# ctxnn/GenConViT

Measured on AMD Instinct MI355X. Metric: frames/sec (224x224, ed+vae forward), higher is better.
Workload: dtype f16

## Files before the change

genconvit_amd/_lib.py:

```python
from __future__ import annotations

import ctypes
import ctypes.util
import json
import os
import threading

_HERE = os.path.dirname(os.path.abspath(__file__))
LIB_PATH = os.environ.get("GCV_LIB_PATH") or os.path.join(_HERE, "lib", "libgenconvit_hip.so")

GCV_F32, GCV_BF16, GCV_F16 = 0, 1, 2
ACT_NONE, ACT_RELU, ACT_GELU, ACT_LEAKY = 0, 1, 2, 3
A_PLAIN, A_IM2COL3_POOL, A_IM2COL3_S2 = 0, 1, 2
EPI_BIAS_ACT, EPI_RESID, EPI_POOL4, EPI_CONVT, EPI_SPLITK = 0, 1, 2, 3, 4

c_void_p, c_int, c_int64, c_float, c_char_p, c_size_t = (ctypes.c_void_p, ctypes.c_int, ctypes.c_int64,
                                                         ctypes.c_float, ctypes.c_char_p, ctypes.c_size_t)


class TensorDesc(ctypes.Structure):
    _fields_ = [("name", c_char_p), ("data", c_void_p), ("numel", c_int64), ("on_device", c_int)]


class GemmArgs(ctypes.Structure):
# ... 95 lines not shown
    "gcv_k_gelu_bwd": (c_int, [c_int, c_void_p, c_void_p, c_void_p, c_void_p, c_int, c_int, c_void_p]),
    "gcv_k_dw_ln_bwd": (c_int, [c_int, c_void_p, c_void_p, c_void_p, c_void_p, c_void_p, c_void_p, c_void_p, c_int, c_int,
                                c_int, c_float, c_void_p]),
    "gcv_k_dw_dgrad_res": (c_int, [c_void_p, c_void_p, c_void_p, c_int, c_int, c_int, c_void_p]),
    "gcv_k_down_ln_bwd": (c_int, [c_int, c_void_p, c_void_p, c_void_p, c_void_p, c_void_p, c_int, c_int, c_int, c_float,
                                  c_void_p]),
    "gcv_k_cam2": (c_int, [c_int, c_int, c_int, c_void_p, c_void_p, c_void_p, c_void_p, c_int, c_int, c_int, c_int, c_int,
                           c_int, c_void_p, c_void_p, c_void_p, c_int, c_void_p]),
    "gcv_k_fused_mlp": (c_int, [c_int, c_int, c_void_p, c_void_p, c_void_p, c_void_p, c_void_p, c_void_p, c_void_p,
                                c_void_p, c_int, c_void_p]),
    "gcv_k_fused_mlp_lnp": (c_int, [c_int, c_int, c_void_p, c_void_p, c_void_p, c_void_p, c_void_p, c_void_p, c_void_p,
                                    c_void_p, c_void_p, c_float, c_int, c_void_p, c_void_p, c_void_p, c_void_p, c_void_p,
                                    c_int, c_void_p]),
    "gcv_k_fused_mlp_timed": (c_int, [c_int, c_int, c_void_p, c_void_p, c_void_p, c_void_p, c_void_p, c_void_p,
                                      c_void_p, c_void_p, c_int, c_int, c_void_p, c_void_p]),
}

_lib = None
_lock = threading.Lock()


class GenConViTHipError(RuntimeError):
    pass


def _preload_hip_runtime():
    cands = []
    try:
        import torch
        cands.append(os.path.join(os.path.dirname(torch.__file__), "lib", "libamdhip64.so"))
# ... 779 lines not shown
```

genconvit_amd/csrc/api.hip:

```cpp
#include "../../include/genconvit_hip.h"

#include <dlfcn.h>

#include <cstdio>
#include <cstdlib>
#include <cstring>
#include <map>
#include <mutex>
#include <set>
#include <sstream>
#include <vector>

#include "cam.h"
#include "cam_bwd.h"
#include "cnx_mlp.h"
#include "gemm.h"
#include "kernels.h"
#include "net.h"

namespace gcv {
static thread_local std::string g_err;
void set_error(const std::string& msg) { g_err = msg; }
const char* get_error() { return g_err.c_str(); }

// ... 132 lines not shown
    GCV_REQUIRE(w[i].name && w[i].data && w[i].numel > 0, "tensor descriptor with null name/data");
    m[w[i].name] = TensorRef{(const float*)w[i].data, w[i].numel, w[i].on_device != 0};
  }
  return 0;
}

template <typename T> struct MlpTestRunner {
  hipStream_t s;
  const char* only;
  template <class F> int run(const char* tag, double, double, F&& f) { return only && std::strcmp(tag, only) ? 0 : f(); }
  int gemm(const char*, const GemmArgs& g, int a_mode, int epi) { return launch_gemm<T>(g, a_mode, epi, s); }
};
template <typename T>
static int k_mlp_dispatch(int C, const void* x, const void* w1, const float* b1, const float* w2_f32, const float* b2,
                          const float* gamma, const void* resid, void* out, int M, hipStream_t s, int iters = 0,
                          float* ms = nullptr, const LnpSpec* lnp = nullptr) {
  struct Bufs {
    hipStream_t s;
    std::vector<void*> p;
    ~Bufs() { (void)hipStreamSynchronize(s); for (void* q : p) (void)hipFree(q); }
  } bufs{s, {}};
  auto alloc = [&](size_t n) -> void* {
    void* q = nullptr;
    if (hipMalloc(&q, n) != hipSuccess) return nullptr;
    bufs.p.push_back(q);
    return q;
  };
  struct Ev {
    hipEvent_t e = nullptr;
    ~Ev() { if (e) (void)hipEventDestroy(e); }
  };
  CnxMlpW<T> w;
  w.kind = mlp_kind(sizeof(T), C);
  GCV_REQUIRE(w.kind != MlpKind::Gemm, "the fused MLP kernels cover C = 96, 192 and 384");
  w.w1 = (const T*)w1; w.b1 = b1; w.b2 = b2; w.gamma = gamma;
  GCV_TRY(pack_cnx_mlp<T>(w, C, w2_f32, alloc, s));
  T* hidden = w.kind == MlpKind::Pair384 ? (T*)alloc(mlp_pair_hidden_bytes(M, C)) : nullptr;
  GCV_REQUIRE(hidden || w.kind != MlpKind::Pair384, "hipMalloc of the hidden tensor");
  auto launch = [&](const char* only) {
    MlpTestRunner<T> r{s, only};
    return launch_cnx_mlp<T>(r, w, C, (const T*)x, (const T*)resid, (T*)out, hidden, M, lnp, s);
  };
  auto timed = [&](const char* only, float* avg) -> int {
    if (iters <= 0) return launch(only);
    Ev e0, e1;
    GCV_CHECK_HIP(hipEventCreate(&e0.e));
    GCV_CHECK_HIP(hipEventCreate(&e1.e));
    GCV_TRY(launch(only));
    GCV_CHECK_HIP(hipEventRecord(e0.e, s));
    for (int i = 0; i < iters; ++i) GCV_TRY(launch(only));
    GCV_CHECK_HIP(hipEventRecord(e1.e, s));
    GCV_CHECK_HIP(hipEventSynchronize(e1.e));
    float t = 0.0f;
    GCV_CHECK_HIP(hipEventElapsedTime(&t, e0.e, e1.e));
    if (avg) *avg = t / (float)iters;
    return 0;
// ... 619 lines not shown
  return launch_face_quality((const unsigned char*)frames_u8_nhwc, nframes, H, W, boxes5, n, grid, out8, (hipStream_t)s);
}

int gcv_face_signature(const void* frames_u8_nhwc, int nframes, int H, int W, const int* boxes5, int n, void* sig384,
                       gcv_stream s) {
  GCV_REQUIRE(n <= 0 || (frames_u8_nhwc && boxes5 && sig384), "face signature: null pointer");
  return launch_face_signature((const unsigned char*)frames_u8_nhwc, nframes, H, W, boxes5, n, (unsigned char*)sig384,
                               (hipStream_t)s);
}

int gcv_sig_link(const void* sig384, const int* owner, int n, int tracks, uint32_t* out_u32, gcv_stream s) {
  GCV_REQUIRE(n <= 0 || tracks <= 0 || (sig384 && owner && out_u32), "sig link: null pointer");
  return launch_sig_link((const unsigned char*)sig384, owner, n, tracks, out_u32, (hipStream_t)s);
}

int gcv_k_fused_mlp(int dtype, int C, const void* x, const void* w1, const float* b1, const float* w2_f32,
                    const float* b2, const float* gamma, const void* resid, void* out, int M, gcv_stream s) {
  GCV_REQUIRE(dtype == GCV_F16 || dtype == GCV_BF16, "the MLP kernels are built for 16-bit storage");
  if (dtype == GCV_F16) return k_mlp_dispatch<half_t>(C, x, w1, b1, w2_f32, b2, gamma, resid, out, M, (hipStream_t)s);
  return k_mlp_dispatch<bf16_t>(C, x, w1, b1, w2_f32, b2, gamma, resid, out, M, (hipStream_t)s);
}

int gcv_k_fused_mlp_lnp(int dtype, int C, const void* x, const void* w1, const float* b1, const float* w2_f32,
                        const float* b2, const float* gamma, const void* resid, const float* ln_w, const float* ln_b,
                        float eps, int nseg, const int* tok0, const int* hw, const int* wd, const int* out0, void* out, int M,
                        gcv_stream s) {
  GCV_REQUIRE(dtype == GCV_F16 || dtype == GCV_BF16, "the MLP kernels are built for 16-bit storage");
  LnpSpec l;
  GCV_TRY(lnp_from_tables(l, C, M, ln_w, ln_b, eps, nseg, tok0, hw, wd, out0));
  if (dtype == GCV_F16)
    return k_mlp_dispatch<half_t>(C, x, w1, b1, w2_f32, b2, gamma, resid, out, M, (hipStream_t)s, 0, nullptr, &l);
  return k_mlp_dispatch<bf16_t>(C, x, w1, b1, w2_f32, b2, gamma, resid, out, M, (hipStream_t)s, 0, nullptr, &l);
}

int gcv_k_fused_mlp_timed(int dtype, int C, const void* x, const void* w1, const float* b1, const float* w2_f32,
                          const float* b2, const float* gamma, const void* resid, void* out, int M, int iters,
                          float* ms3, gcv_stream s) {
  GCV_REQUIRE(dtype == GCV_F16 || dtype == GCV_BF16, "the MLP kernels are built for 16-bit storage");
  GCV_REQUIRE(iters >= 1 && ms3 != nullptr, "gcv_k_fused_mlp_timed: iters >= 1 and a float[3] for the averages");
  if (dtype == GCV_F16)
    return k_mlp_dispatch<half_t>(C, x, w1, b1, w2_f32, b2, gamma, resid, out, M, (hipStream_t)s, iters, ms3);
  return k_mlp_dispatch<bf16_t>(C, x, w1, b1, w2_f32, b2, gamma, resid, out, M, (hipStream_t)s, iters, ms3);
}

}
```

genconvit_amd/csrc/cnx_mlp.h:

```cpp
#pragma once
#include "fused_mlp.h"
#include "gemm.h"
#include "mlp_pair.h"
#include "xs_mlp.h"

namespace gcv {

enum class MlpKind {
  Gemm,
  Fused96,
  Xs192,
  Pair384,
};
static inline MlpKind mlp_kind(size_t tsize, int C) {
  if (tsize != 2) return MlpKind::Gemm;
  if (C == 96) return MlpKind::Fused96;
  if (C == 192) return MlpKind::Xs192;
  if (C == 384) return MlpKind::Pair384;
  return MlpKind::Gemm;
}

template <typename T> struct CnxMlpW {
  MlpKind kind = MlpKind::Gemm;
  const T* w1 = nullptr;
// ... 51 lines not shown
    t += (int64_t)n[s] * h[s] * wd[s];
    o += (int64_t)n[s] * (h[s] / 2) * (wd[s] / 2);
    even = even && h[s] % 2 == 0 && wd[s] % 2 == 0;
  }
  return even && lnp_supported(kind, C, M);
}
template <typename A> static void set_lnp(A& a, const LnpSpec& l) {
  a.lnp_w = l.w; a.lnp_b = l.b; a.lnp_eps = l.eps; a.lnp_nseg = l.nseg;
  for (int s = 0; s < l.nseg; ++s) {
    a.lnp_tok0[s] = l.tok0[s]; a.lnp_hw[s] = l.hw[s]; a.lnp_wd[s] = l.wd[s]; a.lnp_out0[s] = l.out0[s];
  }
}

template <typename T, class R>
int launch_cnx_mlp(R& r, const CnxMlpW<T>& w, int C, const T* x, const T* resid, T* out, T* hidden, int M,
                   const LnpSpec* lnp, hipStream_t s) {
  GCV_REQUIRE(!lnp || lnp_supported(w.kind, C, M), "LN-patchify epilogue of an MLP kind without one");
  if constexpr (sizeof(T) == 2) {
    const double fused_flops = 16.0 * M * C * (double)C, fused_bytes = 3.0 * sizeof(T) * (double)M * C + 16.0 * C * C;
    switch (w.kind) {
      case MlpKind::Gemm: break;
      case MlpKind::Fused96: {
        MlpArgs a{x, w.w1, w.b1, w.w2c, w.b2, w.gamma, resid, out, M};
        if (lnp) set_lnp(a, *lnp);
        return r.run("cnx.fused_mlp", fused_flops, fused_bytes, [&] { return launch_fused_mlp<T>(a, C, s); });
      }
      case MlpKind::Xs192: {
        XsMlpArgs a{x, w.wp, w.b1, w.b2, w.gamma, resid, out, M};
        if (lnp) set_lnp(a, *lnp);
        return r.run("cnx.fused_mlp", fused_flops, fused_bytes, [&] { return launch_xs_mlp<T>(a, C, s); });
      }
      case MlpKind::Pair384: {
        MlpPairArgs a{x, w.w1f, w.b1, w.w2f, w.b2, w.gamma, resid, out, hidden, M};
        GCV_TRY(r.run("cnx.pw1_gelu", 8.0 * M * C * (double)C, sizeof(T) * (5.0 * M * C + 4.0 * C * C),
                      [&] { return launch_xs_pw1<T>(a, C, s); }));
        return r.run("cnx.pw2_scale_res", 8.0 * M * C * (double)C, sizeof(T) * (6.0 * M * C + 4.0 * C * C),
                     [&] { return launch_pw2f<T>(a, C, s); });
      }
    }
  }
  GemmArgs g1{};
  g1.A = x; g1.lda = C; g1.Wt = w.w1; g1.C = hidden; g1.ldc = 4 * C; g1.bias = w.b1;
  g1.M = M; g1.N = 4 * C; g1.K = C; g1.act = ACT_GELU; g1.splitk = 1;
  GCV_TRY(r.gemm("cnx.pw1_gelu", g1, A_PLAIN, EPI_BIAS_ACT));
  GemmArgs g2{};
// ... 7 lines not shown
```

genconvit_amd/csrc/diag/diag.h:

```cpp
#pragma once

#ifndef GCV_XS_ABLATE
#define GCV_XS_ABLATE 0
#endif
#ifndef GCV_P2_ABLATE
#define GCV_P2_ABLATE 0
#endif
#ifndef GCV_XM_ABLATE
#define GCV_XM_ABLATE 0
#endif
#ifndef GCV_MLP_ABLATE
#define GCV_MLP_ABLATE 0
#endif
#ifndef GCV_GLDS_ABLATE
#define GCV_GLDS_ABLATE 0
#endif
#ifndef GCV_DWR_ABLATE
#define GCV_DWR_ABLATE 0
#endif
#ifndef GCV_DWM_ABLATE
#define GCV_DWM_ABLATE 0
#endif
#ifndef GCV_XS_STAMPS
#define GCV_XS_STAMPS 0
#endif
#ifndef GCV_XS_STAMP_WAVE
#define GCV_XS_STAMP_WAVE 0
#endif
#ifndef GCV_P2_STAMPS
#define GCV_P2_STAMPS 0
#endif
#ifndef GCV_P2_STAMP_WAVE
#define GCV_P2_STAMP_WAVE 0
#endif
#ifndef GCV_XM_STAMPS
#define GCV_XM_STAMPS 0
// ... 97 lines not shown
```

genconvit_amd/csrc/fused_mlp.h:

```cpp
#pragma once
#include "gemm.h"

namespace gcv {


struct MlpArgs {
  const void* X;
  const void* W1;
  const float* b1;
  const void* W2c;
  const float* b2;
  const float* gamma;
  const void* resid;
  void* out;
  int M;
  const float* lnp_w = nullptr;
  const float* lnp_b = nullptr;
  float lnp_eps = 0.0f;
  int lnp_nseg = 0;
  int lnp_tok0[4] = {0, 0, 0, 0};
  int lnp_hw[4] = {1, 1, 1, 1};
  int lnp_wd[4] = {1, 1, 1, 1};
  int lnp_out0[4] = {0, 0, 0, 0};
};
// ... 214 lines not shown
    for (int i = 0; i < 12; ++i) {
      const int idx = lane + 64 * i;
      const int row = idx / 24, pc = idx - row * 24;
      const int64_t mm = m_wave + row;
      const f32x4 v = *(const f32x4*)(sC + row * 100 + 4 * pc);
      t4 o4;
#pragma unroll
      for (int e = 0; e < 4; ++e) o4[e] = from_f<T>(v[e] + to_f(rres[i][e]));
      if (mm < a.M) *(t4*)(Op + mm * C + half * 96 + 4 * pc) = o4;
    }
    __syncthreads();
  }
  GCV_STAMP(6);
}

template <typename T> int launch_fused_mlp(const MlpArgs& a, int C, hipStream_t s);
template <typename T> int launch_pack_w2_chunks(const float* w2_dev, T* out, int C, hipStream_t s);

}
```

genconvit_amd/csrc/fused_mlp_bf16.hip:

```cpp
#include "fused_mlp_impl.h"
namespace gcv {
template int launch_fused_mlp<bf16_t>(const MlpArgs&, int, hipStream_t);
template int launch_pack_w2_chunks<bf16_t>(const float*, bf16_t*, int, hipStream_t);
}
```

genconvit_amd/csrc/fused_mlp_f16.hip:

```cpp
#include "fused_mlp_impl.h"
namespace gcv {
template int launch_fused_mlp<half_t>(const MlpArgs&, int, hipStream_t);
template int launch_pack_w2_chunks<half_t>(const float*, half_t*, int, hipStream_t);
}

GCV_MLP_STAMP_READER
```

genconvit_amd/csrc/fused_mlp_impl.h:

```cpp
#pragma once
#include "fused_mlp.h"
#include "fused_mlp_res.h"

namespace gcv {

template <typename T>
__global__ void __launch_bounds__(256) pack_w2_chunks_kernel(const float* __restrict__ w2, T* __restrict__ out, int C,
                                                             int HC) {
  const int64_t total = (int64_t)C * 4 * C;
  const int64_t i = (int64_t)blockIdx.x * 256 + threadIdx.x;
  if (i >= total) return;
  const int p = (int)(i % HC);
  const int64_t t = i / HC;
  const int o = (int)(t % C);
  const int ch = (int)(t / C);
  const int kk = p >> 4, h = (p >> 3) & 1, jj = p & 7;
  const int hid = 16 * kk + 8 * (jj >> 2) + 4 * h + (jj & 3);
  out[i] = from_f<T>(w2[(int64_t)o * 4 * C + ch * HC + hid]);
}

template <typename T> int launch_pack_w2_chunks(const float* w2_dev, T* out, int C, hipStream_t s) {
  constexpr int HC = kMlpHC;
  GCV_REQUIRE((4 * C) % HC == 0, "hidden width must be a multiple of the chunk");
  const int64_t total = (int64_t)C * 4 * C;
  hipLaunchKernelGGL((pack_w2_chunks_kernel<T>), dim3((unsigned)cdiv64(total, 256)), dim3(256), 0, s, w2_dev, out, C, HC);
  GCV_CHECK_HIP(hipGetLastError());
  return 0;
}

template <typename T, int C, int NW> static int launch_mlp_c(const MlpArgs& a, hipStream_t s) {
  constexpr int SMEM = MlpSmem<T, C, NW>::bytes;
  GCV_ENSURE_LDS((fused_mlp_kernel<T, C, NW>), SMEM);
  hipLaunchKernelGGL((fused_mlp_kernel<T, C, NW>), dim3(cdiv(a.M, NW * 32)), dim3(NW * 64), SMEM, s, a);
  GCV_CHECK_HIP(hipGetLastError());
  return 0;
}

template <typename T> int launch_fused_mlp_res(const MlpArgs& a, hipStream_t s) {
  constexpr int SMEM = MlpResSmem::bytes;
  GCV_ENSURE_LDS((fused_mlp_res_kernel<T>), SMEM);
  constexpr int nw = 8;
  const int wave_tiles = cdiv(a.M, 32);
  const int nwg = cdiv(wave_tiles, nw) < 256 ? cdiv(wave_tiles, nw) : 256;
  if (a.lnp_nseg > 0) {
    GCV_REQUIRE(a.lnp_w && a.lnp_b && a.lnp_nseg <= 4, "fused MLP: LN-patchify epilogue arguments");
    GCV_ENSURE_LDS((fused_mlp_res_kernel<T, true>), SMEM);
    hipLaunchKernelGGL((fused_mlp_res_kernel<T, true>), dim3(nwg), dim3(64 * nw), SMEM, s, a);
  } else {
    hipLaunchKernelGGL((fused_mlp_res_kernel<T>), dim3(nwg), dim3(64 * nw), SMEM, s, a);
  }
  GCV_CHECK_HIP(hipGetLastError());
  return 0;
}

template <typename T> int launch_fused_mlp(const MlpArgs& a, int C, hipStream_t s) {
  GCV_REQUIRE(a.M > 0 && a.X && a.W1 && a.W2c && a.b1 && a.b2 && a.gamma && a.resid && a.out, "fused MLP: null argument");
  if (fused_mlp_res_applies(C, a.M)) return launch_fused_mlp_res<T>(a, s);
  GCV_REQUIRE(a.lnp_nseg == 0, "fused MLP: the LN-patchify epilogue exists in the LDS-resident kernel only");
  GCV_REQUIRE(C == 96, "fused MLP kernels of this file: C = 96");
  return launch_mlp_c<T, 96, 4>(a, s);
}

}
```

genconvit_amd/csrc/fused_mlp_res.h:

```cpp
#pragma once
#include "fused_mlp.h"

namespace gcv {

struct MlpResSmem {
  static constexpr int kRow = 192;
  static constexpr int kW1 = 0;
  static constexpr int kW2 = 384 * kRow;
  static constexpr int kB1 = 2 * 384 * kRow;
  static constexpr int kB2 = kB1 + 384 * 4;
  static constexpr int kG = kB2 + 96 * 4;
  static constexpr int kCtr = kG + 96 * 4;
  static constexpr int kLn = kCtr + 16;
  static constexpr int bytes = kLn + 2 * 96 * 4;
};

__device__ __forceinline__ int mlp_res_swz(int row, int k16) { return (k16 & ~3) | ((k16 & 3) ^ ((row >> 2) & 3)); }

template <typename T, bool LNP = false>
__global__ void __launch_bounds__(512, 1) fused_mlp_res_kernel(const MlpArgs a) {
  static_assert(sizeof(T) == 2, "fused MLP is built for 16-bit storage");
  constexpr int C = 96, HC = 96, NG = 12;
  constexpr int KP1 = C / 16;
  constexpr int NO = C / 32;
// ... 25 lines not shown
      sf[i] = i < 384 ? a.b1[i] : (i < 480 ? a.b2[i - 384] : a.gamma[i - 480]);
    if (tid == 0) *reinterpret_cast<int*>(smem + MlpResSmem::kCtr) = (int)blockDim.x >> 6;
    if (LNP) {
      float* sl = reinterpret_cast<float*>(smem + MlpResSmem::kLn);
      for (int i = tid; i < 192; i += (int)blockDim.x) sl[i] = i < 96 ? a.lnp_w[i] : a.lnp_b[i - 96];
    }
  }
  __syncthreads();
  RES_STAMP(11);

  const T* __restrict__ Xp = (const T*)a.X;
  const T* Rp = (const T*)a.resid;
  T* Op = (T*)a.out;
  typedef T t4 __attribute__((ext_vector_type(4)));

  const int ntiles = (a.M + 31) / 32;
  const int nwaves = (int)blockDim.x >> 6;
  const int stride = (int)gridDim.x * nwaves;
  const int key = (lr >> 2) & 3;
  const int rowoff = lr * ROW;

  u32x4 xf[KP1];
  auto load_x = [&](int tile) {
    const int64_t mm = (int64_t)tile * 32 + lr;
    const int64_t mmc = (GCV_MLP_ABLATE & 8) ? (int64_t)lr : (mm < a.M ? mm : (int64_t)a.M - 1);
#pragma unroll
    for (int p = 0; p < KP1; ++p) xf[p] = *(const u32x4*)(Xp + mmc * C + 16 * p + 8 * lh);
  };
  int* const ctr = reinterpret_cast<int*>(smem + MlpResSmem::kCtr);
  auto slot_tile = [&](int q) { return (int)blockIdx.x * nwaves + (q % nwaves) + (q / nwaves) * stride; };
  auto next_slot = [&]() {
    int q = 0;
    if (lane == 0) q = atomicAdd(ctr, 1);
    return __builtin_amdgcn_readfirstlane(q);
  };
  if (slot_tile(wave) < ntiles) load_x(slot_tile(wave));
  int titer = 0;
  for (int tile = slot_tile(wave), tile_next = 0; tile < ntiles; tile = tile_next, ++titer) {
    tile_next = slot_tile(next_slot());
    if (titer == 2) GCV_STAMP(0);
#if GCV_MLP_STAMPS
    if (titer == 2 && blockIdx.x < 64 && threadIdx.x == 0) gcv_mlp_stamps[blockIdx.x * 16 + 8] = __builtin_amdgcn_s_memrealtime();
#endif
    const int64_t m = (int64_t)tile * 32 + lr;
    const int64_t mc = m < a.M ? m : (int64_t)a.M - 1;
// ... 209 lines not shown
        }
        auto sx = __builtin_amdgcn_permlane32_swap(pk[0].x, pk[1].x, false, false);
        auto sy = __builtin_amdgcn_permlane32_swap(pk[0].y, pk[1].y, false, false);
        const u32x4 w = {sx[0], sy[0], sx[1], sy[1]};
        const int n16 = 32 * o + 8 * q + 8 * lh;
        if (m < a.M && (!(GCV_MLP_ABLATE & 8) || w[0] == 0x12345u)) *(u32x4*)(Op + m * C + n16) = w;
      }
    if (titer == 2) GCV_STAMP(6);
#if GCV_MLP_STAMPS
    if (titer == 2 && blockIdx.x < 64 && threadIdx.x == 0) gcv_mlp_stamps[blockIdx.x * 16 + 9] = __builtin_amdgcn_s_memrealtime();
#endif
  }
  RES_STAMP(12);
}

template <typename T> int launch_fused_mlp_res(const MlpArgs& a, hipStream_t s);

}
```

genconvit_amd/csrc/xs_mlp.h:

```cpp
#pragma once
#include <type_traits>

#include "gemm.h"

namespace gcv {

struct XsMlpArgs {
  const void* X;
  const void* Wp;
  const float* b1;
  const float* b2;
  const float* gamma;
  const void* resid;
  void* out;
  int M;
  const float* lnp_w = nullptr;
  const float* lnp_b = nullptr;
  float lnp_eps = 0.0f;
  int lnp_nseg = 0;
  int lnp_tok0[4] = {0, 0, 0, 0};
  int lnp_hw[4] = {1, 1, 1, 1};
  int lnp_wd[4] = {1, 1, 1, 1};
  int lnp_out0[4] = {0, 0, 0, 0};
};
// ... 25 lines not shown
  static constexpr int NKC = 4 * C / 32;
  static constexpr int D = C == 96 ? 10 : 6;
  static constexpr int PPW = 3;
  static constexpr int NLW = NM / PPW;
  static constexpr int kB1 = D * REC;
  static constexpr int kBG = kB1 + 4 * C * 4;
  static constexpr int kLn = kBG + 2 * C * 4;
  static constexpr int bytes = kLn + 2 * C * 4;
  static constexpr int NSB = NM / 4;
};


#define GCV_XM_WAIT(N) asm volatile("s_waitcnt vmcnt(%0)\n\ts_barrier" ::"n"(N) : "memory")

template <typename T, int C, bool LNP = false>
__global__ void __launch_bounds__(512, 2) xs_mlp_kernel(const XsMlpArgs a, const int npass) {
  static_assert(sizeof(T) == 2, "16-bit storage");
  static_assert(C == 96 || C == 192, "narrow ConvNeXt stages");
  typedef XsMlpCfg<C> CF;
  constexpr int KP1 = CF::KP1, NO = CF::NO, NM = CF::NM, REC = CF::REC, NKC = CF::NKC, D = CF::D, PPW = CF::PPW;
  constexpr int NLW = CF::NLW, NSB = CF::NSB;
  static_assert(D >= 6 && NKC % 2 == 0, "ring: four live chunks and two incoming; passes are whole pairs of steps");
  typedef T t4 __attribute__((ext_vector_type(4)));

  extern __shared__ __attribute__((aligned(16))) unsigned char smem[];

  const int tid = threadIdx.x;
  const int lane = tid & 63;
  const int wave = __builtin_amdgcn_readfirstlane(tid >> 6);
  const int lr = lane & 31, lh = lane >> 5;

  const int my_passes = (npass - (int)blockIdx.x + (int)gridDim.x - 1) / (int)gridDim.x;
  if (my_passes <= 0) return;

  {
    float* sf = reinterpret_cast<float*>(smem + CF::kB1);
    for (int i = tid; i < 6 * C; i += 512) sf[i] = i < 4 * C ? a.b1[i] : (i < 5 * C ? a.b2[i - 4 * C] : a.gamma[i - 5 * C]);
    if (LNP) {
      float* sl = reinterpret_cast<float*>(smem + CF::kLn);
      for (int i = tid; i < 2 * C; i += 512) sl[i] = i < C ? a.lnp_w[i] : a.lnp_b[i - C];
    }
  }
  __syncthreads();

  const bool loader = wave < NLW;
  const unsigned char* const wsrc = (const unsigned char*)a.Wp + wave * 1024;
  const unsigned lane16 = (unsigned)lane * 16u;
  int gw = 0, slot_w = 0;
  auto issue = [&]() {
    if (loader) {
      const unsigned char* src = wsrc + (int64_t)gw * REC;
      unsigned char* dst = smem + slot_w * REC + wave * 1024;
#pragma unroll
      for (int i = 0; i < PPW; ++i)
        __builtin_amdgcn_global_load_lds((const __attribute__((address_space(1))) void*)(src + i * NLW * 1024 + lane16),
                                         (__attribute__((address_space(3))) void*)(dst + i * NLW * 1024), 16, 0, 0);
    }
    gw = gw + 1 == NKC ? 0 : gw + 1;
    slot_w = slot_w + 1 == D ? 0 : slot_w + 1;
  };
// ... 5 lines not shown
  const float* const sG_ = sB2_ + C;
  const T* __restrict__ Xp = (const T*)a.X;
  const T* Rp = (const T*)a.resid;
  T* Op = (T*)a.out;

  int slot1 = 0;
  auto slot_dec = [&](int s, int k) { return s - k < 0 ? s - k + D : s - k; };

  u32x4 xf[KP1];
  auto load_x = [&](int64_t mc) {
    const T* xp = Xp + mc * C + 8 * lh;
#pragma unroll
    for (int p = 0; p < KP1; ++p)
      asm volatile("global_load_dwordx4 %0, %1, off offset:%2" : "=v"(xf[p]) : "v"(xp), "n"(p * 32) : "memory");
  };
  auto row_of = [&](int it) { return ((int64_t)((int)blockIdx.x + it * (int)gridDim.x) * 8 + wave) * 32 + lr; };
  {
    const int64_t m0 = row_of(0);
    load_x(m0 < a.M ? m0 : (int64_t)a.M - 1);
  }
  XM_STAMP(0);

  for (int it = 0; it < my_passes; ++it) {
    const int64_t m = row_of(it);
    const int64_t mc = m < a.M ? m : (int64_t)a.M - 1;
    asm volatile("s_waitcnt vmcnt(0)" ::: "memory");
#pragma unroll
    for (int p = 0; p < KP1; ++p) asm volatile("" : "+v"(xf[p]));

    f32x16 acc2[NO];
#pragma unroll
    for (int o = 0; o < NO; ++o)
#pragma unroll
      for (int r = 0; r < 16; ++r) acc2[o][r] = 0.0f;

    GeluH16::State<4> gst;
    float gx[8];
    auto gelu_a = [&](const f32x16& acc, int half) {
#pragma unroll
      for (int c = 0; c < 8; ++c) gx[c] = acc[8 * half + c];
// ... 198 lines not shown
            const int q = 2 * pr + d;
            const int n = 32 * o + 8 * q;
            const f32x4 bv = *(const f32x4*)(sB2 + n);
            const f32x4 gv = *(const f32x4*)(sG + n);
            t4 o4;
#pragma unroll
            for (int e = 0; e < 4; ++e) o4[e] = from_f<T>(fmaf(acc2[o][4 * q + e] + bv[e], gv[e], to_f(rq[d][e])));
            pk[d] = __builtin_bit_cast(uint2, o4);
          }
          const auto sx = __builtin_amdgcn_permlane32_swap(pk[0].x, pk[1].x, false, false);
          const auto sy = __builtin_amdgcn_permlane32_swap(pk[0].y, pk[1].y, false, false);
          const u32x4 w = {sx[0], sy[0], sx[1], sy[1]};
          if (m < a.M) *(u32x4*)(Op + m * C + 32 * o + 16 * pr + 8 * lh) = w;
        }
    }
    if (it + 1 < my_passes) {
      const int64_t mn = row_of(it + 1);
      load_x(mn < a.M ? mn : (int64_t)a.M - 1);
    }
    if (it == 0) XM_STAMP(5);
  }
  asm volatile("s_waitcnt vmcnt(0)" ::: "memory");
  XM_STAMP(6);
}

template <typename T> int launch_xs_mlp(const XsMlpArgs& a, int C, hipStream_t s);
template <typename T, typename S> int launch_pack_xs_mlp(const T* w1, const S* w2, T* out, int C, hipStream_t s);
static inline bool xs_mlp_supported(int C) { return C == 192; }
static inline size_t xs_mlp_packed_elems(int C) { return (size_t)(4 * C / 32) * (size_t)(C / 16 + 2 * (C / 32)) * 512; }

}
```

genconvit_amd/csrc/xs_mlp_bf16.hip:

```cpp
#include "xs_mlp_impl.h"
namespace gcv {
template int launch_xs_mlp<bf16_t>(const XsMlpArgs&, int, hipStream_t);
template int launch_pack_xs_mlp<bf16_t, bf16_t>(const bf16_t*, const bf16_t*, bf16_t*, int, hipStream_t);
template int launch_pack_xs_mlp<bf16_t, float>(const bf16_t*, const float*, bf16_t*, int, hipStream_t);
}
```

genconvit_amd/csrc/xs_mlp_f16.hip:

```cpp
#include "xs_mlp_impl.h"
namespace gcv {
template int launch_xs_mlp<half_t>(const XsMlpArgs&, int, hipStream_t);
template int launch_pack_xs_mlp<half_t, half_t>(const half_t*, const half_t*, half_t*, int, hipStream_t);
template int launch_pack_xs_mlp<half_t, float>(const half_t*, const float*, half_t*, int, hipStream_t);
}

GCV_XM_STAMP_READER
```

genconvit_amd/csrc/xs_mlp_impl.h:

```cpp
#pragma once
#include "xs_mlp.h"

namespace gcv {

template <typename T, typename S> int launch_pack_xs_mlp(const T* w1, const S* w2, T* out, int C, hipStream_t s) {
  GCV_REQUIRE(xs_mlp_supported(C), "pack_xs_mlp: unsupported C");
  const int64_t total = (int64_t)xs_mlp_packed_elems(C);
  hipLaunchKernelGGL((pack_xs_mlp_kernel<T, S>), dim3((unsigned)cdiv64(total, 256)), dim3(256), 0, s, w1, w2, out, C);
  GCV_CHECK_HIP(hipGetLastError());
  return 0;
}

template <typename T, int C> static int launch_xs_mlp_c(const XsMlpArgs& a, hipStream_t s) {
  constexpr int SMEM = XsMlpCfg<C>::bytes;
  GCV_ENSURE_LDS((xs_mlp_kernel<T, C>), SMEM);
  const int npass = cdiv(a.M, 256);
  const int nwg = npass < 256 ? npass : 256;
  if (a.lnp_nseg > 0) {
    GCV_REQUIRE(a.lnp_w && a.lnp_b && a.lnp_nseg <= 4, "xs MLP: LN-patchify epilogue arguments");
    GCV_ENSURE_LDS((xs_mlp_kernel<T, C, true>), SMEM);
    hipLaunchKernelGGL((xs_mlp_kernel<T, C, true>), dim3(nwg), dim3(512), SMEM, s, a, npass);
    GCV_CHECK_HIP(hipGetLastError());
    return 0;
  }
  hipLaunchKernelGGL((xs_mlp_kernel<T, C>), dim3(nwg), dim3(512), SMEM, s, a, npass);
  GCV_CHECK_HIP(hipGetLastError());
  return 0;
}

template <typename T> int launch_xs_mlp(const XsMlpArgs& a, int C, hipStream_t s) {
  GCV_REQUIRE(a.M > 0 && a.X && a.Wp && a.b1 && a.b2 && a.gamma && a.resid && a.out, "xs MLP: null argument");
  auto al = [](const void* p) { return (reinterpret_cast<uintptr_t>(p) & 15u) == 0; };
  GCV_REQUIRE(al(a.X) && al(a.Wp) && al(a.resid) && al(a.out), "xs MLP: operands must be 16-byte aligned");
  if (C == 192) return launch_xs_mlp_c<T, 192>(a, s);
  set_error("xs MLP is built for C = 192");
  return -3;
}

}
```

include/genconvit_hip.h:

```cpp
#ifndef GENCONVIT_HIP_H
#define GENCONVIT_HIP_H

#include <stddef.h>
#include <stdint.h>

#ifdef __cplusplus
extern "C" {
#endif

#if defined(GCV_BUILD)
#pragma GCC visibility push(default)
#endif

typedef struct gcv_handle gcv_handle;
typedef void* gcv_stream;

enum { GCV_F32 = 0, GCV_BF16 = 1, GCV_F16 = 2 };
enum { GCV_CONVNEXT_TINY = 0, GCV_CONVNEXT_LARGE = 1 };
enum { GCV_LARGE_MAX_BATCH = 256 };
enum { GCV_ACT_NONE = 0, GCV_ACT_RELU = 1, GCV_ACT_GELU = 2, GCV_ACT_LEAKY = 3 };

typedef struct {
  const char* name;
  const void* data;
// ... 162 lines not shown
int gcv_k_down_ln_bwd(int dtype, const void* x, const float* ln_w, const float* dP, const float* inv, float* dA2,
                      int nimg, int side2, int C2, float eps, gcv_stream s);
int gcv_k_cam2(int dtype, int C2, int npass, const void* A0, const void* A1, const float* dA0, const float* dA1,
               int side0, int side1, int off0, int off1, int cam_ld, int up_pass, float* cam, float* cam224, float* alpha,
               int B, gcv_stream s);

int gcv_k_fused_mlp(int dtype, int C, const void* x, const void* w1, const float* b1, const float* w2_f32,
                    const float* b2, const float* gamma, const void* resid, void* out, int M, gcv_stream s);
int gcv_k_fused_mlp_lnp(int dtype, int C, const void* x, const void* w1, const float* b1, const float* w2_f32,
                        const float* b2, const float* gamma, const void* resid, const float* ln_w, const float* ln_b,
                        float eps, int nseg, const int* tok0, const int* hw, const int* wd, const int* out0, void* out, int M,
                        gcv_stream s);
int gcv_k_fused_mlp_timed(int dtype, int C, const void* x, const void* w1, const float* b1, const float* w2_f32,
                          const float* b2, const float* gamma, const void* resid, void* out, int M, int iters,
                          float* ms3, gcv_stream s);

#if defined(GCV_BUILD)
#pragma GCC visibility pop
#endif

#ifdef __cplusplus
}
#endif
#endif
```

Baseline: 18580.

## Spread MLP tail tiles across workgroups with a shared tile-walk scheme

Adds a shared tile-walk helper that both fused MLP kernels (C=96 LDS-resident and C=192 xs) use to map tiles to workgroup waves. The partial last round is spread across more workgroups instead of being packed onto the first few, so the tail imbalance shrinks. In the xs kernel, waves that finish early keep issuing weight-stream loads so the shared loader pipeline stays in step. It also exposes max-workgroup entry points and a walk-inspection API for testing. The cost is extra per-kernel index arithmetic and idle loader loops.

```diff
diff --git a/genconvit_amd/_lib.py b/genconvit_amd/_lib.py
--- a/genconvit_amd/_lib.py
+++ b/genconvit_amd/_lib.py
@@ -133,6 +133,12 @@
                                     c_int, c_void_p]),
     "gcv_k_fused_mlp_timed": (c_int, [c_int, c_int, c_void_p, c_void_p, c_void_p, c_void_p, c_void_p, c_void_p,
                                       c_void_p, c_void_p, c_int, c_int, c_void_p, c_void_p]),
+    "gcv_k_fused_mlp_wg": (c_int, [c_int, c_int, c_void_p, c_void_p, c_void_p, c_void_p, c_void_p, c_void_p, c_void_p,
+                                   c_void_p, c_int, c_int, c_void_p]),
+    "gcv_k_fused_mlp_lnp_wg": (c_int, [c_int, c_int, c_void_p, c_void_p, c_void_p, c_void_p, c_void_p, c_void_p, c_void_p,
+                                       c_void_p, c_void_p, c_float, c_int, c_void_p, c_void_p, c_void_p, c_void_p, c_void_p,
+                                       c_int, c_int, c_void_p]),
+    "gcv_mlp_walk": (c_int, [c_int, c_int, c_int, c_void_p, c_void_p, c_int]),
 }
 
 _lib = None
diff --git a/genconvit_amd/csrc/api.hip b/genconvit_amd/csrc/api.hip
--- a/genconvit_amd/csrc/api.hip
+++ b/genconvit_amd/csrc/api.hip
@@ -170,7 +170,7 @@
 template <typename T>
 static int k_mlp_dispatch(int C, const void* x, const void* w1, const float* b1, const float* w2_f32, const float* b2,
                           const float* gamma, const void* resid, void* out, int M, hipStream_t s, int iters = 0,
-                          float* ms = nullptr, const LnpSpec* lnp = nullptr) {
+                          float* ms = nullptr, const LnpSpec* lnp = nullptr, int max_wg = kMlpMaxWg) {
   struct Bufs {
     hipStream_t s;
     std::vector<void*> p;
@@ -195,7 +195,7 @@
   GCV_REQUIRE(hidden || w.kind != MlpKind::Pair384, "hipMalloc of the hidden tensor");
   auto launch = [&](const char* only) {
     MlpTestRunner<T> r{s, only};
-    return launch_cnx_mlp<T>(r, w, C, (const T*)x, (const T*)resid, (T*)out, hidden, M, lnp, s);
+    return launch_cnx_mlp<T>(r, w, C, (const T*)x, (const T*)resid, (T*)out, hidden, M, lnp, s, max_wg);
   };
   auto timed = [&](const char* only, float* avg) -> int {
     if (iters <= 0) return launch(only);
@@ -845,23 +845,56 @@
   return launch_sig_link((const unsigned char*)sig384, owner, n, tracks, out_u32, (hipStream_t)s);
 }
 
+int gcv_k_fused_mlp_wg(int dtype, int C, const void* x, const void* w1, const float* b1, const float* w2_f32,
+                       const float* b2, const float* gamma, const void* resid, void* out, int M, int max_wg, gcv_stream s) {
+  GCV_REQUIRE(dtype == GCV_F16 || dtype == GCV_BF16, "the MLP kernels are built for 16-bit storage");
+  GCV_REQUIRE(max_wg >= 1 && max_wg <= kMlpMaxWg, "fused MLP: max_wg outside 1 .. 256");
+  if (dtype == GCV_F16)
+    return k_mlp_dispatch<half_t>(C, x, w1, b1, w2_f32, b2, gamma, resid, out, M, (hipStream_t)s, 0, nullptr, nullptr, max_wg);
+  return k_mlp_dispatch<bf16_t>(C, x, w1, b1, w2_f32, b2, gamma, resid, out, M, (hipStream_t)s, 0, nullptr, nullptr, max_wg);
+}
+
 int gcv_k_fused_mlp(int dtype, int C, const void* x, const void* w1, const float* b1, const float* w2_f32,
                     const float* b2, const float* gamma, const void* resid, void* out, int M, gcv_stream s) {
+  return gcv_k_fused_mlp_wg(dtype, C, x, w1, b1, w2_f32, b2, gamma, resid, out, M, kMlpMaxWg, s);
+}
+
+int gcv_k_fused_mlp_lnp_wg(int dtype, int C, const void* x, const void* w1, const float* b1, const float* w2_f32,
+                           const float* b2, const float* gamma, const void* resid, const float* ln_w, const float* ln_b,
+                           float eps, int nseg, const int* tok0, const int* hw, const int* wd, const int* out0, void* out,
+                           int M, int max_wg, gcv_stream s) {
   GCV_REQUIRE(dtype == GCV_F16 || dtype == GCV_BF16, "the MLP kernels are built for 16-bit storage");
-  if (dtype == GCV_F16) return k_mlp_dispatch<half_t>(C, x, w1, b1, w2_f32, b2, gamma, resid, out, M, (hipStream_t)s);
-  return k_mlp_dispatch<bf16_t>(C, x, w1, b1, w2_f32, b2, gamma, resid, out, M, (hipStream_t)s);
+  GCV_REQUIRE(max_wg >= 1 && max_wg <= kMlpMaxWg, "fused MLP: max_wg outside 1 .. 256");
+  LnpSpec l;
+  GCV_TRY(lnp_from_tables(l, C, M, ln_w, ln_b, eps, nseg, tok0, hw, wd, out0));
+  if (dtype == GCV_F16)
+    return k_mlp_dispatch<half_t>(C, x, w1, b1, w2_f32, b2, gamma, resid, out, M, (hipStream_t)s, 0, nullptr, &l, max_wg);
+  return k_mlp_dispatch<bf16_t>(C, x, w1, b1, w2_f32, b2, gamma, resid, out, M, (hipStream_t)s, 0, nullptr, &l, max_wg);
 }
 
 int gcv_k_fused_mlp_lnp(int dtype, int C, const void* x, const void* w1, const float* b1, const float* w2_f32,
                         const float* b2, const float* gamma, const void* resid, const float* ln_w, const float* ln_b,
                         float eps, int nseg, const int* tok0, const int* hw, const int* wd, const int* out0, void* out, int M,
                         gcv_stream s) {
-  GCV_REQUIRE(dtype == GCV_F16 || dtype == GCV_BF16, "the MLP kernels are built for 16-bit storage");
-  LnpSpec l;
-  GCV_TRY(lnp_from_tables(l, C, M, ln_w, ln_b, eps, nseg, tok0, hw, wd, out0));
-  if (dtype == GCV_F16)
-    return k_mlp_dispatch<half_t>(C, x, w1, b1, w2_f32, b2, gamma, resid, out, M, (hipStream_t)s, 0, nullptr, &l);
-  return k_mlp_dispatch<bf16_t>(C, x, w1, b1, w2_f32, b2, gamma, resid, out, M, (hipStream_t)s, 0, nullptr, &l);
+  return gcv_k_fused_mlp_lnp_wg(dtype, C, x, w1, b1, w2_f32, b2, gamma, resid, ln_w, ln_b, eps, nseg, tok0, hw, wd, out0, out,
+                                M, kMlpMaxWg, s);
+}
+
+int gcv_mlp_walk(int C, int M, int G, int* out3, int* tiles, int ntile_slots) {
+  GCV_REQUIRE(out3 && (C == 96 || C == 192) && M >= 1 && G >= 1 && G <= kMlpMaxWg,
+              "gcv_mlp_walk: C = 96 or 192, M >= 1, 1 .. 256 workgroups");
+  const MlpWalk w = mlp_walk(C, M, G);
+  out3[0] = w.full; out3[1] = w.tail; out3[2] = w.spread;
+  if (!tiles) return 0;
+  const int64_t need = (int64_t)(w.full + 1) * G * kMlpWalkSlots;
+  GCV_REQUIRE(ntile_slots >= need, "gcv_mlp_walk: tiles holds fewer than (full + 1) * G * 8 entries");
+  for (int r = 0; r <= w.full; ++r)
+    for (int wg = 0; wg < G; ++wg)
+      for (int k = 0; k < kMlpWalkSlots; ++k) {
+        const int t = mlp_walk_tile(w, C, wg, k, r);
+        tiles[((int64_t)r * G + wg) * kMlpWalkSlots + k] = t < w.ntiles ? t : -1;
+      }
+  return 0;
 }
 
 int gcv_k_fused_mlp_timed(int dtype, int C, const void* x, const void* w1, const float* b1, const float* w2_f32,
diff --git a/genconvit_amd/csrc/cnx_mlp.h b/genconvit_amd/csrc/cnx_mlp.h
--- a/genconvit_amd/csrc/cnx_mlp.h
+++ b/genconvit_amd/csrc/cnx_mlp.h
@@ -89,7 +89,7 @@
 
 template <typename T, class R>
 int launch_cnx_mlp(R& r, const CnxMlpW<T>& w, int C, const T* x, const T* resid, T* out, T* hidden, int M,
-                   const LnpSpec* lnp, hipStream_t s) {
+                   const LnpSpec* lnp, hipStream_t s, int max_wg = kMlpMaxWg) {
   GCV_REQUIRE(!lnp || lnp_supported(w.kind, C, M), "LN-patchify epilogue of an MLP kind without one");
   if constexpr (sizeof(T) == 2) {
     const double fused_flops = 16.0 * M * C * (double)C, fused_bytes = 3.0 * sizeof(T) * (double)M * C + 16.0 * C * C;
@@ -98,12 +98,12 @@
       case MlpKind::Fused96: {
         MlpArgs a{x, w.w1, w.b1, w.w2c, w.b2, w.gamma, resid, out, M};
         if (lnp) set_lnp(a, *lnp);
-        return r.run("cnx.fused_mlp", fused_flops, fused_bytes, [&] { return launch_fused_mlp<T>(a, C, s); });
+        return r.run("cnx.fused_mlp", fused_flops, fused_bytes, [&] { return launch_fused_mlp<T>(a, C, s, max_wg); });
       }
       case MlpKind::Xs192: {
         XsMlpArgs a{x, w.wp, w.b1, w.b2, w.gamma, resid, out, M};
         if (lnp) set_lnp(a, *lnp);
-        return r.run("cnx.fused_mlp", fused_flops, fused_bytes, [&] { return launch_xs_mlp<T>(a, C, s); });
+        return r.run("cnx.fused_mlp", fused_flops, fused_bytes, [&] { return launch_xs_mlp<T>(a, C, s, max_wg); });
       }
       case MlpKind::Pair384: {
         MlpPairArgs a{x, w.w1f, w.b1, w.w2f, w.b2, w.gamma, resid, out, hidden, M};
diff --git a/genconvit_amd/csrc/diag/diag.h b/genconvit_amd/csrc/diag/diag.h
--- a/genconvit_amd/csrc/diag/diag.h
+++ b/genconvit_amd/csrc/diag/diag.h
@@ -20,6 +20,9 @@
 #endif
 #ifndef GCV_DWM_ABLATE
 #define GCV_DWM_ABLATE 0
+#endif
+#ifndef GCV_XM_TAIL_WAVES
+#define GCV_XM_TAIL_WAVES 4
 #endif
 #ifndef GCV_XS_STAMPS
 #define GCV_XS_STAMPS 0
diff --git a/genconvit_amd/csrc/fused_mlp.h b/genconvit_amd/csrc/fused_mlp.h
--- a/genconvit_amd/csrc/fused_mlp.h
+++ b/genconvit_amd/csrc/fused_mlp.h
@@ -1,5 +1,6 @@
 #pragma once
 #include "gemm.h"
+#include "mlp_walk.h"
 
 namespace gcv {
 
@@ -252,7 +253,7 @@
   GCV_STAMP(6);
 }
 
-template <typename T> int launch_fused_mlp(const MlpArgs& a, int C, hipStream_t s);
+template <typename T> int launch_fused_mlp(const MlpArgs& a, int C, hipStream_t s, int max_wg = kMlpMaxWg);
 template <typename T> int launch_pack_w2_chunks(const float* w2_dev, T* out, int C, hipStream_t s);
 
 }
diff --git a/genconvit_amd/csrc/fused_mlp_bf16.hip b/genconvit_amd/csrc/fused_mlp_bf16.hip
--- a/genconvit_amd/csrc/fused_mlp_bf16.hip
+++ b/genconvit_amd/csrc/fused_mlp_bf16.hip
@@ -1,5 +1,5 @@
 #include "fused_mlp_impl.h"
 namespace gcv {
-template int launch_fused_mlp<bf16_t>(const MlpArgs&, int, hipStream_t);
+template int launch_fused_mlp<bf16_t>(const MlpArgs&, int, hipStream_t, int);
 template int launch_pack_w2_chunks<bf16_t>(const float*, bf16_t*, int, hipStream_t);
 }
diff --git a/genconvit_amd/csrc/fused_mlp_f16.hip b/genconvit_amd/csrc/fused_mlp_f16.hip
--- a/genconvit_amd/csrc/fused_mlp_f16.hip
+++ b/genconvit_amd/csrc/fused_mlp_f16.hip
@@ -1,6 +1,6 @@
 #include "fused_mlp_impl.h"
 namespace gcv {
-template int launch_fused_mlp<half_t>(const MlpArgs&, int, hipStream_t);
+template int launch_fused_mlp<half_t>(const MlpArgs&, int, hipStream_t, int);
 template int launch_pack_w2_chunks<half_t>(const float*, half_t*, int, hipStream_t);
 }
 
diff --git a/genconvit_amd/csrc/fused_mlp_impl.h b/genconvit_amd/csrc/fused_mlp_impl.h
--- a/genconvit_amd/csrc/fused_mlp_impl.h
+++ b/genconvit_amd/csrc/fused_mlp_impl.h
@@ -36,12 +36,12 @@
   return 0;
 }
 
-template <typename T> int launch_fused_mlp_res(const MlpArgs& a, hipStream_t s) {
+template <typename T> int launch_fused_mlp_res(const MlpArgs& a, hipStream_t s, int max_wg) {
   constexpr int SMEM = MlpResSmem::bytes;
   GCV_ENSURE_LDS((fused_mlp_res_kernel<T>), SMEM);
-  constexpr int nw = 8;
-  const int wave_tiles = cdiv(a.M, 32);
-  const int nwg = cdiv(wave_tiles, nw) < 256 ? cdiv(wave_tiles, nw) : 256;
+  GCV_REQUIRE(max_wg >= 1 && max_wg <= kMlpMaxWg, "fused MLP: 1 .. 256 workgroups");
+  constexpr int nw = kMlpWalkSlots;
+  const int nwg = mlp_walk_grid(a.M, max_wg);
   if (a.lnp_nseg > 0) {
     GCV_REQUIRE(a.lnp_w && a.lnp_b && a.lnp_nseg <= 4, "fused MLP: LN-patchify epilogue arguments");
     GCV_ENSURE_LDS((fused_mlp_res_kernel<T, true>), SMEM);
@@ -53,9 +53,9 @@
   return 0;
 }
 
-template <typename T> int launch_fused_mlp(const MlpArgs& a, int C, hipStream_t s) {
+template <typename T> int launch_fused_mlp(const MlpArgs& a, int C, hipStream_t s, int max_wg) {
   GCV_REQUIRE(a.M > 0 && a.X && a.W1 && a.W2c && a.b1 && a.b2 && a.gamma && a.resid && a.out, "fused MLP: null argument");
-  if (fused_mlp_res_applies(C, a.M)) return launch_fused_mlp_res<T>(a, s);
+  if (fused_mlp_res_applies(C, a.M)) return launch_fused_mlp_res<T>(a, s, max_wg);
   GCV_REQUIRE(a.lnp_nseg == 0, "fused MLP: the LN-patchify epilogue exists in the LDS-resident kernel only");
   GCV_REQUIRE(C == 96, "fused MLP kernels of this file: C = 96");
   return launch_mlp_c<T, 96, 4>(a, s);
diff --git a/genconvit_amd/csrc/fused_mlp_res.h b/genconvit_amd/csrc/fused_mlp_res.h
--- a/genconvit_amd/csrc/fused_mlp_res.h
+++ b/genconvit_amd/csrc/fused_mlp_res.h
@@ -63,9 +63,8 @@
   T* Op = (T*)a.out;
   typedef T t4 __attribute__((ext_vector_type(4)));
 
-  const int ntiles = (a.M + 31) / 32;
-  const int nwaves = (int)blockDim.x >> 6;
-  const int stride = (int)gridDim.x * nwaves;
+  const MlpWalk wk = mlp_walk(C, a.M, (int)gridDim.x);
+  const int ntiles = wk.ntiles;
   const int key = (lr >> 2) & 3;
   const int rowoff = lr * ROW;
 
@@ -77,7 +76,9 @@
     for (int p = 0; p < KP1; ++p) xf[p] = *(const u32x4*)(Xp + mmc * C + 16 * p + 8 * lh);
   };
   int* const ctr = reinterpret_cast<int*>(smem + MlpResSmem::kCtr);
-  auto slot_tile = [&](int q) { return (int)blockIdx.x * nwaves + (q % nwaves) + (q / nwaves) * stride; };
+  auto slot_tile = [&](int q) {
+    return mlp_walk_tile(wk, C, (int)blockIdx.x, q % kMlpWalkSlots, q / kMlpWalkSlots);
+  };
   auto next_slot = [&]() {
     int q = 0;
     if (lane == 0) q = atomicAdd(ctr, 1);
@@ -317,6 +318,6 @@
   RES_STAMP(12);
 }
 
-template <typename T> int launch_fused_mlp_res(const MlpArgs& a, hipStream_t s);
+template <typename T> int launch_fused_mlp_res(const MlpArgs& a, hipStream_t s, int max_wg = kMlpMaxWg);
 
 }
diff --git a/genconvit_amd/csrc/mlp_walk.h b/genconvit_amd/csrc/mlp_walk.h
--- /dev/null
+++ b/genconvit_amd/csrc/mlp_walk.h
@@ -0,0 +1,64 @@
+#pragma once
+#include "diag/diag.h"
+
+#if defined(__HIPCC__) || defined(__CUDACC__)
+#define GCV_WALK_HD __host__ __device__
+#else
+#define GCV_WALK_HD
+#endif
+
+namespace gcv {
+
+constexpr int kMlpWalkSlots = 8;
+constexpr int kMlpWalkSpread192 = GCV_XM_TAIL_WAVES;
+constexpr int kMlpMaxWg = 256;
+
+struct MlpWalk {
+  int G;
+  int ntiles;
+  int full;
+  int tail;
+  int spread;
+};
+
+GCV_WALK_HD static inline MlpWalk mlp_walk(int C, int M, int G) {
+  MlpWalk w;
+  w.G = G;
+  w.ntiles = (M + 31) / 32;
+  const int round = kMlpWalkSlots * G;
+  w.full = w.ntiles / round;
+  w.tail = w.ntiles - w.full * round;
+  if (C == 192) {
+    const int t = (w.tail + kMlpWalkSlots - 1) / kMlpWalkSlots;
+    w.spread = t > 0 && 2 * t <= G && (w.tail + kMlpWalkSpread192 - 1) / kMlpWalkSpread192 <= G;
+  } else {
+    w.spread = w.tail > 0 && w.tail <= 4 * G;
+  }
+  return w;
+}
+
+GCV_WALK_HD static inline int mlp_walk_tile(const MlpWalk& w, int C, int wg, int k, int r) {
+  if (r > w.full) return w.ntiles;
+  int tile;
+  if (r < w.full || !w.spread) {
+    tile = (wg + r * w.G) * kMlpWalkSlots + k;
+  } else if (C == 192) {
+    if (k >= kMlpWalkSpread192) return w.ntiles;
+    tile = w.full * w.G * kMlpWalkSlots + wg * kMlpWalkSpread192 + k;
+  } else {
+    tile = w.full * w.G * kMlpWalkSlots + wg + k * w.G;
+  }
+  return tile < w.ntiles ? tile : w.ntiles;
+}
+
+GCV_WALK_HD static inline int mlp_walk_slot_rounds(const MlpWalk& w, int C, int wg, int k) {
+  return w.full + (mlp_walk_tile(w, C, wg, k, w.full) < w.ntiles ? 1 : 0);
+}
+GCV_WALK_HD static inline int mlp_walk_rounds(const MlpWalk& w, int C, int wg) { return mlp_walk_slot_rounds(w, C, wg, 0); }
+
+static inline int mlp_walk_grid(int M, int max_wg) {
+  const int passes = (M + 32 * kMlpWalkSlots - 1) / (32 * kMlpWalkSlots);
+  return passes < max_wg ? passes : max_wg;
+}
+
+}
diff --git a/genconvit_amd/csrc/xs_mlp.h b/genconvit_amd/csrc/xs_mlp.h
--- a/genconvit_amd/csrc/xs_mlp.h
+++ b/genconvit_amd/csrc/xs_mlp.h
@@ -2,6 +2,7 @@
 #include <type_traits>
 
 #include "gemm.h"
+#include "mlp_walk.h"
 
 namespace gcv {
 
@@ -63,7 +64,7 @@
 #define GCV_XM_WAIT(N) asm volatile("s_waitcnt vmcnt(%0)\n\ts_barrier" ::"n"(N) : "memory")
 
 template <typename T, int C, bool LNP = false>
-__global__ void __launch_bounds__(512, 2) xs_mlp_kernel(const XsMlpArgs a, const int npass) {
+__global__ void __launch_bounds__(512, 2) xs_mlp_kernel(const XsMlpArgs a) {
   static_assert(sizeof(T) == 2, "16-bit storage");
   static_assert(C == 96 || C == 192, "narrow ConvNeXt stages");
   typedef XsMlpCfg<C> CF;
@@ -79,8 +80,13 @@
   const int wave = __builtin_amdgcn_readfirstlane(tid >> 6);
   const int lr = lane & 31, lh = lane >> 5;
 
-  const int my_passes = (npass - (int)blockIdx.x + (int)gridDim.x - 1) / (int)gridDim.x;
+  MlpWalk wk = mlp_walk(C, a.M, (int)gridDim.x);
+  wk.full = __builtin_amdgcn_readfirstlane(wk.full);
+  wk.spread = __builtin_amdgcn_readfirstlane(wk.spread);
+  const int my_passes = __builtin_amdgcn_readfirstlane(mlp_walk_rounds(wk, C, (int)blockIdx.x));
   if (my_passes <= 0) return;
+  const int my_tiles = __builtin_amdgcn_readfirstlane(mlp_walk_slot_rounds(wk, C, (int)blockIdx.x, wave));
+  const int idle_pairs = __builtin_amdgcn_readfirstlane((my_passes - my_tiles) * (NKC / 2));
 
   {
     float* sf = reinterpret_cast<float*>(smem + CF::kB1);
@@ -92,7 +98,7 @@
   }
   __syncthreads();
 
-  const bool loader = wave < NLW;
+  const bool loader = NLW >= 8 || wave < NLW;
   const unsigned char* const wsrc = (const unsigned char*)a.Wp + wave * 1024;
   const unsigned lane16 = (unsigned)lane * 16u;
   int gw = 0, slot_w = 0;
@@ -128,16 +134,16 @@
     for (int p = 0; p < KP1; ++p)
       asm volatile("global_load_dwordx4 %0, %1, off offset:%2" : "=v"(xf[p]) : "v"(xp), "n"(p * 32) : "memory");
   };
-  auto row_of = [&](int it) { return ((int64_t)((int)blockIdx.x + it * (int)gridDim.x) * 8 + wave) * 32 + lr; };
-  {
-    const int64_t m0 = row_of(0);
-    load_x(m0 < a.M ? m0 : (int64_t)a.M - 1);
-  }
+  auto tile_of = [&](int it) { return mlp_walk_tile(wk, C, (int)blockIdx.x, wave, it); };
+  auto row_of = [&](int tile) { return (int64_t)tile * 32 + lr; };
+  auto clamp_row = [&](int64_t m) { return m < a.M ? m : (int64_t)a.M - 1; };
+  int tile = tile_of(0);
+  load_x(clamp_row(row_of(tile)));
   XM_STAMP(0);
 
-  for (int it = 0; it < my_passes; ++it) {
-    const int64_t m = row_of(it);
-    const int64_t mc = m < a.M ? m : (int64_t)a.M - 1;
+  for (int it = 0; it < my_tiles; ++it) {
+    const int64_t m = row_of(tile);
+    const int64_t mc = clamp_row(m);
     asm volatile("s_waitcnt vmcnt(0)" ::: "memory");
 #pragma unroll
     for (int p = 0; p < KP1; ++p) asm volatile("" : "+v"(xf[p]));
@@ -366,17 +372,22 @@
           if (m < a.M) *(u32x4*)(Op + m * C + 32 * o + 16 * pr + 8 * lh) = w;
         }
     }
-    if (it + 1 < my_passes) {
-      const int64_t mn = row_of(it + 1);
-      load_x(mn < a.M ? mn : (int64_t)a.M - 1);
+    if (it + 1 < my_tiles) {
+      tile = tile_of(it + 1);
+      load_x(clamp_row(row_of(tile)));
     }
     if (it == 0) XM_STAMP(5);
+  }
+#pragma unroll 1
+  for (int g = idle_pairs; g > 0; --g) {
+    GCV_XM_WAIT(0);
+    if (!(GCV_XM_ABLATE & 2)) { issue(); issue(); }
   }
   asm volatile("s_waitcnt vmcnt(0)" ::: "memory");
   XM_STAMP(6);
 }
 
-template <typename T> int launch_xs_mlp(const XsMlpArgs& a, int C, hipStream_t s);
+template <typename T> int launch_xs_mlp(const XsMlpArgs& a, int C, hipStream_t s, int max_wg = kMlpMaxWg);
 template <typename T, typename S> int launch_pack_xs_mlp(const T* w1, const S* w2, T* out, int C, hipStream_t s);
 static inline bool xs_mlp_supported(int C) { return C == 192; }
 static inline size_t xs_mlp_packed_elems(int C) { return (size_t)(4 * C / 32) * (size_t)(C / 16 + 2 * (C / 32)) * 512; }
diff --git a/genconvit_amd/csrc/xs_mlp_bf16.hip b/genconvit_amd/csrc/xs_mlp_bf16.hip
--- a/genconvit_amd/csrc/xs_mlp_bf16.hip
+++ b/genconvit_amd/csrc/xs_mlp_bf16.hip
@@ -1,6 +1,6 @@
 #include "xs_mlp_impl.h"
 namespace gcv {
-template int launch_xs_mlp<bf16_t>(const XsMlpArgs&, int, hipStream_t);
+template int launch_xs_mlp<bf16_t>(const XsMlpArgs&, int, hipStream_t, int);
 template int launch_pack_xs_mlp<bf16_t, bf16_t>(const bf16_t*, const bf16_t*, bf16_t*, int, hipStream_t);
 template int launch_pack_xs_mlp<bf16_t, float>(const bf16_t*, const float*, bf16_t*, int, hipStream_t);
 }
diff --git a/genconvit_amd/csrc/xs_mlp_f16.hip b/genconvit_amd/csrc/xs_mlp_f16.hip
--- a/genconvit_amd/csrc/xs_mlp_f16.hip
+++ b/genconvit_amd/csrc/xs_mlp_f16.hip
@@ -1,6 +1,6 @@
 #include "xs_mlp_impl.h"
 namespace gcv {
-template int launch_xs_mlp<half_t>(const XsMlpArgs&, int, hipStream_t);
+template int launch_xs_mlp<half_t>(const XsMlpArgs&, int, hipStream_t, int);
 template int launch_pack_xs_mlp<half_t, half_t>(const half_t*, const half_t*, half_t*, int, hipStream_t);
 template int launch_pack_xs_mlp<half_t, float>(const half_t*, const float*, half_t*, int, hipStream_t);
 }
diff --git a/genconvit_amd/csrc/xs_mlp_impl.h b/genconvit_amd/csrc/xs_mlp_impl.h
--- a/genconvit_amd/csrc/xs_mlp_impl.h
+++ b/genconvit_amd/csrc/xs_mlp_impl.h
@@ -11,28 +11,28 @@
   return 0;
 }
 
-template <typename T, int C> static int launch_xs_mlp_c(const XsMlpArgs& a, hipStream_t s) {
+template <typename T, int C> static int launch_xs_mlp_c(const XsMlpArgs& a, hipStream_t s, int max_wg) {
   constexpr int SMEM = XsMlpCfg<C>::bytes;
   GCV_ENSURE_LDS((xs_mlp_kernel<T, C>), SMEM);
-  const int npass = cdiv(a.M, 256);
-  const int nwg = npass < 256 ? npass : 256;
+  const int nwg = mlp_walk_grid(a.M, max_wg);
   if (a.lnp_nseg > 0) {
     GCV_REQUIRE(a.lnp_w && a.lnp_b && a.lnp_nseg <= 4, "xs MLP: LN-patchify epilogue arguments");
     GCV_ENSURE_LDS((xs_mlp_kernel<T, C, true>), SMEM);
-    hipLaunchKernelGGL((xs_mlp_kernel<T, C, true>), dim3(nwg), dim3(512), SMEM, s, a, npass);
+    hipLaunchKernelGGL((xs_mlp_kernel<T, C, true>), dim3(nwg), dim3(512), SMEM, s, a);
     GCV_CHECK_HIP(hipGetLastError());
     return 0;
   }
-  hipLaunchKernelGGL((xs_mlp_kernel<T, C>), dim3(nwg), dim3(512), SMEM, s, a, npass);
+  hipLaunchKernelGGL((xs_mlp_kernel<T, C>), dim3(nwg), dim3(512), SMEM, s, a);
   GCV_CHECK_HIP(hipGetLastError());
   return 0;
 }
 
-template <typename T> int launch_xs_mlp(const XsMlpArgs& a, int C, hipStream_t s) {
+template <typename T> int launch_xs_mlp(const XsMlpArgs& a, int C, hipStream_t s, int max_wg) {
   GCV_REQUIRE(a.M > 0 && a.X && a.Wp && a.b1 && a.b2 && a.gamma && a.resid && a.out, "xs MLP: null argument");
+  GCV_REQUIRE(max_wg >= 1 && max_wg <= kMlpMaxWg, "xs MLP: 1 .. 256 workgroups");
   auto al = [](const void* p) { return (reinterpret_cast<uintptr_t>(p) & 15u) == 0; };
   GCV_REQUIRE(al(a.X) && al(a.Wp) && al(a.resid) && al(a.out), "xs MLP: operands must be 16-byte aligned");
-  if (C == 192) return launch_xs_mlp_c<T, 192>(a, s);
+  if (C == 192) return launch_xs_mlp_c<T, 192>(a, s, max_wg);
   set_error("xs MLP is built for C = 192");
   return -3;
 }
diff --git a/include/genconvit_hip.h b/include/genconvit_hip.h
--- a/include/genconvit_hip.h
+++ b/include/genconvit_hip.h
@@ -200,6 +200,13 @@
 int gcv_k_fused_mlp_timed(int dtype, int C, const void* x, const void* w1, const float* b1, const float* w2_f32,
                           const float* b2, const float* gamma, const void* resid, void* out, int M, int iters,
                           float* ms3, gcv_stream s);
+int gcv_k_fused_mlp_wg(int dtype, int C, const void* x, const void* w1, const float* b1, const float* w2_f32,
+                       const float* b2, const float* gamma, const void* resid, void* out, int M, int max_wg, gcv_stream s);
+int gcv_k_fused_mlp_lnp_wg(int dtype, int C, const void* x, const void* w1, const float* b1, const float* w2_f32,
+                           const float* b2, const float* gamma, const void* resid, const float* ln_w, const float* ln_b,
+                           float eps, int nseg, const int* tok0, const int* hw, const int* wd, const int* out0, void* out,
+                           int M, int max_wg, gcv_stream s);
+int gcv_mlp_walk(int C, int M, int G, int* out3, int* tiles, int ntile_slots);
 
 #if defined(GCV_BUILD)
 #pragma GCC visibility pop
```

Result: no change. 18680, median of 6 (+0.6%).
